# T1uTiu/ProDiff

Measured on AMD Instinct MI355X. Metric: mel-frames/sec + audio RTF, 2-iter ProDiff + 4-iter FastDiff @1/2/4/8 GPU, higher is better.
Workload: dtype bf16; 1 GPU; C3: ProDiff 2-iter (WaveNet 20x256, M=80, vpsde max_beta 40) + FastDiff 4-iter (base.yaml, hop 256), 8 x 861-frame utterances per GPU; global_batch=8, per_gpu_batch=8, seq_len=861, batches_per_gpu=1, jobs_in_flight=2, schedule=job i on HIP stream i % 2, parallelism=dp1 (utterance shards, RCCL gather to rank 0)

## Files before the change

### include/prodiff_hip.h

```cpp
#ifndef PRODIFF_HIP_H
#define PRODIFF_HIP_H

#include <stddef.h>

#ifdef __cplusplus
extern "C" {
#endif

#define PD_OK 0
#define PD_ERR_ARG 1
#define PD_ERR_HIP 2
#define PD_ERR_WORKSPACE 3
#define PD_ERR_UNSUPPORTED 4

#define PD_DTYPE_F32 0
#define PD_DTYPE_BF16 1

const char* pd_last_error(void);
int pd_version(void);
const char* pd_build_config(void);
size_t pd_live_device_bytes(void);

int pd_profile_enable(int on);
int pd_profile_summary(char* buf, int buflen);
// ... 55 lines not shown
  int inner_channels;
  int cond_channels;
  int num_blocks;
  int upsample_ratios[4];
  int lvc_layers_each_block;
  int lvc_kernel_size;
  int kpnet_hidden_channels;
  int kpnet_conv_size;
  int step_embed_in;
  int step_embed_mid;
  int step_embed_out;
} fd_dims;

#define FD_NUM_PARAMS(nb) (2 + 4 + 30 * (nb) + 8 * (nb) + 2)

int fd_create(const fd_dims* dims, const float* const* params, int dtype, void* stream,
              fd_model** out);
void fd_destroy(fd_model* m);
int fd_hop(const fd_model* m);
size_t fd_workspace_size(const fd_model* m, int B, int Tc, int S);

#define FD_OPT_LVC_TS 0
#define FD_OPT_LVC_TS_SUB 1
#define FD_OPT_LVC_FUSE 2
#define FD_OPT_LVC_PF 3
#define FD_OPT_LVC_SUB 4
#define FD_OPT_KP_SIDE 5
#define FD_OPT_KP_CHUNK 7
#define FD_OPT_LVC_TPW 10
#define FD_OPT_LVC_PRIO 11
#define FD_OPT_LVC_PS 14
#define FD_OPT_LVC_CARRY 15
#define FD_OPT_LVC_PS_GRID 16
int fd_set_option(fd_model* m, int option, int value);

int fd_lvc_ps_partition(int rows, int batch, int grid, int* runs, int cap, int* nruns);

int fd_fold_weight_norm(float* w, const float* g, const float* v, int cout, int per_row,
                        void* stream);

int fd_forward(const fd_model* m, const float* audio, const float* cond, const float* steps,
               float* eps, int B, int Tc, void* workspace, size_t ws_bytes, void* stream);

int fd_sample(const fd_model* m, const float* mel, const float* beta, const float* alpha,
              const float* sigma, const float* steps, int N, const float* x_T,
              const float* noise, unsigned long long seed, const int* utt_ids, const int* lens, float* wav,
              int B, int Tc, void* workspace, size_t ws_bytes, void* stream);

int fd_sample_coefs(const fd_model* m, const float* mel, const float* ce, const float* den,
                    const float* sg, const float* steps, int N, const float* x_T,
                    const float* noise, unsigned long long seed, const int* utt_ids, const int* lens,
                    int draw0, float* wav, int B, int Tc, void* workspace, size_t ws_bytes, void* stream);

int fd_draw_x_T(const fd_model* m, float* x_T, int B, int Tc, unsigned long long seed, const int* utt_ids,
                void* stream);

typedef struct nsf_model nsf_model;

typedef struct {
  int num_mels;
  int upsample_initial_channel;
  int num_upsamples;
  int upsample_rates[6];
  int upsample_kernel_sizes[6];
  int resblock;
  int num_kernels;
  int resblock_kernel_sizes[4];
  int num_dilations;
  int resblock_dilation_sizes[4][4];
// ... 278 lines not shown
```

### prodiff_amd/_lib.py

```python
from __future__ import annotations

import ctypes as C
import os

_HERE = os.path.dirname(os.path.abspath(__file__))
LIB_PATH = os.environ.get("PRODIFF_HIP_LIB", os.path.join(_HERE, "libprodiff_hip.so"))

PD_DTYPE_F32 = 0
PD_DTYPE_BF16 = 1
PD_REFLOW = {"euler": 0, "rk2": 1, "rk4": 2, "rk5": 3}
FD_OPTIONS = {"lvc_ts": 0, "lvc_ts_sub": 1, "lvc_fuse": 2, "lvc_pf": 3, "lvc_sub": 4, "kp_side": 5, "kp_chunk": 7,
               "lvc_tpw": 10, "lvc_prio": 11, "lvc_ps": 14, "lvc_carry": 15, "lvc_ps_grid": 16}
NSF_OPTIONS = {"small_max": 0, "wconv": 1, "pair": 2, "pair16": 3, "ups_nc": 4, "rb16": 5, "rb32": 6, "rb64": 7, "c256": 8, "nc_mfma": 9}
WN_OPTIONS = {"layer": 0, "ksplit": 1, "l2pf": 2, "stack": 3, "stack_ro": 4, "stack_fuse": 6, "f32_layer": 7}


class HipError(RuntimeError):
    pass


class pd_wavenet_dims(C.Structure):
    _fields_ = [("in_dims", C.c_int), ("hidden_size", C.c_int), ("residual_layers", C.c_int),
                ("residual_channels", C.c_int), ("dilation_cycle_length", C.c_int)]


class fd_dims(C.Structure):
    _fields_ = [("audio_channels", C.c_int), ("inner_channels", C.c_int),
                ("cond_channels", C.c_int), ("num_blocks", C.c_int),
                ("upsample_ratios", C.c_int * 4), ("lvc_layers_each_block", C.c_int),
                ("lvc_kernel_size", C.c_int), ("kpnet_hidden_channels", C.c_int),
                ("kpnet_conv_size", C.c_int), ("step_embed_in", C.c_int),
                ("step_embed_mid", C.c_int), ("step_embed_out", C.c_int)]


class nsf_dims(C.Structure):
    _fields_ = [("num_mels", C.c_int), ("upsample_initial_channel", C.c_int), ("num_upsamples", C.c_int),
                ("upsample_rates", C.c_int * 6), ("upsample_kernel_sizes", C.c_int * 6), ("resblock", C.c_int),
                ("num_kernels", C.c_int), ("resblock_kernel_sizes", C.c_int * 4), ("num_dilations", C.c_int),
                ("resblock_dilation_sizes", (C.c_int * 4) * 4), ("sampling_rate", C.c_int),
                ("harmonic_num", C.c_int)]


class pd_cond_dims(C.Structure):
    _fields_ = [("vocab_size", C.c_int), ("hidden_size", C.c_int), ("enc_layers", C.c_int),
                ("enc_ffn_kernel_size", C.c_int), ("num_heads", C.c_int), ("num_spk", C.c_int),
# ... 56 lines not shown

class pd_curves_dims(C.Structure):
    _fields_ = [("samplerate", C.c_int), ("win_size", C.c_int), ("hop_size", C.c_int), ("half_width", C.c_float)]


_VP = C.c_void_p
_SIGS = {
    "pd_last_error": (C.c_char_p, []),
    "pd_version": (C.c_int, []),
    "pd_build_config": (C.c_char_p, []),
    "pd_live_device_bytes": (C.c_size_t, []),
    "pd_profile_enable": (C.c_int, [C.c_int]),
    "pd_profile_summary": (C.c_int, [C.c_char_p, C.c_int]),
    "pd_profile_filter": (C.c_int, [C.c_char_p]),
    "pd_wavenet_create": (C.c_int, [C.POINTER(pd_wavenet_dims), C.POINTER(_VP), C.c_int, _VP, C.POINTER(_VP)]),
    "pd_wavenet_destroy": (None, [_VP]),
    "pd_wavenet_set_option": (C.c_int, [_VP, C.c_int, C.c_int]),
    "pd_wavenet_workspace_size": (C.c_size_t, [_VP, C.c_int, C.c_int, C.c_int]),
    "pd_wavenet_forward": (C.c_int, [_VP, _VP, _VP, _VP, _VP, C.c_int, C.c_int, _VP, C.c_size_t, _VP]),
    "pd_prodiff_sample": (C.c_int, [_VP, _VP, C.POINTER(C.c_float), C.POINTER(C.c_float),
                                    C.POINTER(C.c_float), C.c_int, _VP, _VP, C.c_ulonglong, _VP, _VP, _VP,
                                    C.c_int, C.c_int, _VP, C.c_size_t, _VP]),
    "pd_reflow_workspace_size": (C.c_size_t, [_VP, C.c_int, C.c_int, C.c_int, C.c_int]),
    "pd_reflow_sample": (C.c_int, [_VP, _VP, C.c_int, C.c_int, C.c_float, _VP, C.c_ulonglong, _VP, _VP, _VP,
                                   C.c_int, C.c_int, _VP, C.c_size_t, _VP]),
    "pd_reflow_denorm": (C.c_int, [_VP, _VP, _VP, C.c_int, C.c_int, C.c_int, C.c_int, C.c_float, C.c_float,
                                   _VP, _VP]),
    "fd_create": (C.c_int, [C.POINTER(fd_dims), C.POINTER(_VP), C.c_int, _VP, C.POINTER(_VP)]),
    "fd_destroy": (None, [_VP]),
    "fd_hop": (C.c_int, [_VP]),
    "fd_workspace_size": (C.c_size_t, [_VP, C.c_int, C.c_int, C.c_int]),
    "fd_set_option": (C.c_int, [_VP, C.c_int, C.c_int]),
    "fd_lvc_ps_partition": (C.c_int, [C.c_int, C.c_int, C.c_int, C.POINTER(C.c_int), C.c_int, C.POINTER(C.c_int)]),
    "fd_fold_weight_norm": (C.c_int, [_VP, _VP, _VP, C.c_int, C.c_int, _VP]),
    "fd_forward": (C.c_int, [_VP, _VP, _VP, _VP, _VP, C.c_int, C.c_int, _VP, C.c_size_t, _VP]),
    "fd_sample": (C.c_int, [_VP, _VP, C.POINTER(C.c_float), C.POINTER(C.c_float), C.POINTER(C.c_float),
                            C.POINTER(C.c_float), C.c_int, _VP, _VP, C.c_ulonglong, _VP, _VP, _VP, C.c_int,
                            C.c_int, _VP, C.c_size_t, _VP]),
    "fd_sample_coefs": (C.c_int, [_VP, _VP, C.POINTER(C.c_float), C.POINTER(C.c_float), C.POINTER(C.c_float),
                                  C.POINTER(C.c_float), C.c_int, _VP, _VP, C.c_ulonglong, _VP, _VP, C.c_int, _VP,
                                  C.c_int, C.c_int, _VP, C.c_size_t, _VP]),
    "fd_draw_x_T": (C.c_int, [_VP, _VP, C.c_int, C.c_int, C.c_ulonglong, _VP, _VP]),
    "pd_cond_num_params": (C.c_int, [C.POINTER(pd_cond_dims)]),
    "pd_cond_create": (C.c_int, [C.POINTER(pd_cond_dims), C.POINTER(_VP), C.c_int, _VP, C.POINTER(_VP)]),
    "pd_cond_destroy": (None, [_VP]),
    "pd_cond_workspace_size": (C.c_size_t, [_VP, C.c_int, C.c_int, C.c_int]),
    "pd_cond_forward": (C.c_int, [_VP, C.POINTER(pd_cond_inputs), _VP, _VP, C.c_int, C.c_int, C.c_int, _VP,
                                  C.c_size_t, _VP]),
    "pd_pitch_cond_num_params": (C.c_int, [C.POINTER(pd_pitch_cond_dims)]),
    "pd_pitch_cond_create": (C.c_int, [C.POINTER(pd_pitch_cond_dims), C.POINTER(_VP), C.c_int, _VP, C.POINTER(_VP)]),
    "pd_pitch_cond_destroy": (None, [_VP]),
    "pd_pitch_cond_workspace_size": (C.c_size_t, [_VP, C.c_int, C.c_int, C.c_int, C.c_int]),
    "pd_pitch_cond_forward": (C.c_int, [_VP, C.POINTER(pd_pitch_cond_inputs), _VP, C.c_int, C.c_int, C.c_int,
                                        C.c_int, _VP, C.c_size_t, _VP]),
    "pd_dur_num_params": (C.c_int, [C.POINTER(pd_dur_dims)]),
    "pd_dur_create": (C.c_int, [C.POINTER(pd_dur_dims), C.POINTER(_VP), C.c_int, _VP, C.POINTER(_VP)]),
    "pd_dur_destroy": (None, [_VP]),
    "pd_dur_workspace_size": (C.c_size_t, [_VP, C.c_int, C.c_int]),
    "pd_dur_forward": (C.c_int, [_VP, C.POINTER(pd_dur_inputs), _VP, _VP, C.c_int, C.c_int, _VP, C.c_size_t, _VP]),
    "nsf_num_params": (C.c_int, [C.POINTER(nsf_dims)]),
    "nsf_create": (C.c_int, [C.POINTER(nsf_dims), C.POINTER(_VP), C.c_int, _VP, C.POINTER(_VP)]),
    "nsf_destroy": (None, [_VP]),
    "nsf_hop": (C.c_int, [_VP]),
    "nsf_workspace_size": (C.c_size_t, [_VP, C.c_int, C.c_int]),
    "nsf_set_option": (C.c_int, [_VP, C.c_int, C.c_int]),
    "nsf_forward": (C.c_int, [_VP, _VP, C.c_float, _VP, _VP, _VP, C.c_ulonglong, _VP, _VP, _VP, C.c_int, C.c_int,
# ... 349 lines not shown
```

### prodiff_amd/csrc/fastdiff.hip

```cpp
#include <cmath>
#include <vector>

#include "../../include/prodiff_hip.h"
#include "gemm.h"
#include "kernels.h"

using namespace pd;

namespace {
constexpr int CI = 32;
constexpr int CC = 80;
constexpr int HK = 64;
constexpr int NLY = 4;
constexpr int KPERLAYER = 2 * CI * CI * 3;
constexpr int EMB_IN = 128, EMB_MID = 512, EMB_OUT = 512;
constexpr int FD_STEP_CHUNK = 16;

__host__ __device__ inline int lvc_pos(int ci) { return (((ci >> 2) & 1) << 4) | ((ci >> 3) << 2) | (ci & 3); }
__host__ __device__ inline int lvc_chan(int p) { return (p & 3) | (((p & 15) >> 2) << 3) | ((p >> 4) << 2); }
__host__ __device__ inline int kf_packed(int o, int q) {
  const int k = (q & ~31) | lvc_pos(q & 31);
  return (((o >> 5) * 6 + (k >> 4)) * 64 + ((k & 15) >> 3) * 32 + (o & 31)) * 8 + (k & 7);
}
__host__ __device__ inline void kf_unpack(int p, int& o, int& q) {
  const int j = p & 7, l = (p >> 3) & 63, kkn = p >> 9;
  o = (kkn / 6) * 32 + (l & 31);
  const int k = (kkn % 6) * 16 + (l >> 5) * 8 + j;
  q = (k & ~31) | lvc_chan(k & 31);
}
}

struct fd_model {
  int nblocks;
  int ratios[4];
  int hops[4];
  int dtype;
  int lvc_ts = 384;
  int lvc_ts_sub = 256;
  bool lvc_fuse = true;
  bool lvc_pf = true;
  bool lvc_sub = true;
  bool kp_side = false;
  int kp_chunk = 0;
  int lvc_tpw = 2;
  int lvc_prio = 0;
  int lvc_ps = 1;
  int lvc_carry = 1;
  int lvc_ps_grid = 0;

  mutable hipStream_t side = nullptr;
  mutable hipEvent_t ev_hidden = nullptr, ev_kp[4] = {}, ev_lvc[4] = {};
  WeightPool weights;
  DevBuf kps;
  float *fc1_w, *fc1_b, *fc2_w, *fc2_b;
  float *first_w, *first_b;
  float *final_w, *final_b;
  struct Block {
    float *up_w, *up_b;
    float *upf_w;
    float *fct_w, *fct_b;
    float *kin_w, *kin_b;
    float *kres_w[6], *kres_b[6];
    float *kk_w, *kk_b;
    __bf16* kks_w = nullptr;
    float* kks_b = nullptr;
    float *kb_w, *kb_b;
    float *cv_w[NLY], *cv_b[NLY];
  } blk[4];
  struct Down {
    float *c0_w, *c0_b, *c1_w, *c1_b;
    float *c2_w, *c2_b;
  } dn[4];

  ~fd_model() {
    if (side) {
      (void)hipStreamSynchronize(side);
      (void)hipStreamDestroy(side);
    }
    if (ev_hidden) (void)hipEventDestroy(ev_hidden);
    for (int n = 0; n < 4; ++n) {
      if (ev_kp[n]) (void)hipEventDestroy(ev_kp[n]);
// ... 206 lines not shown
      const int s = mt * 32 + (reg & 3) + 8 * (reg >> 2) + 4 * h;
      const long long idx = (base + t0 + s) * CI + r32;
      x[idx] = x[idx] + a[idx] + gate_fast(ag[reg] + bg, afl[reg] + bl);
    }
  }
}

struct LvcBlockArgs {
  float* xout;
  const float* xin;
  const float* a;
  const __bf16* Kf[NLY];
  const float* Bf;
  const __bf16* Wc[NLY];
  const float* bc[NLY];
  const __bf16* Wup;
  const float* bup;
  int r, p;
  const float* audio;
  const float* fw;
  const float* fb;
  const float* wfin;
  const float* bfin;
  float* audio_out;
  const float* noise;
  float ce, den, sig;
  unsigned long long seed;
  unsigned stream;
  const int* uid;
  int Tc, hop;
  const int* lens;
  int b_off;
  int prio;
#ifdef LB_TRACE
  unsigned long long* trace;
#endif
};
#ifdef LB_TRACE
#define LB_STAMP(i)                                                                       \
  do {                                                                                    \
    if (lane == 0 && blockIdx.x % 61 == 0)                                                \
      P.trace[((blockIdx.y * gridDim.x + blockIdx.x) / 61 * NW + wave) * 24 + (i)] =      \
          __builtin_readcyclecounter();                                                   \
  } while (0)
#else
#define LB_STAMP(i) \
  do {              \
  } while (0)
#endif
constexpr int LB_LD = 40;
constexpr int LB_XLD = 36;
template <int TS, int TPW = 2> struct LbGeo {
  static constexpr int NG = TS / 32 + 4;
  static constexpr int NW = NG / TPW;
  static constexpr int NT = NW * 64;
  static constexpr int UOFF = 28;
  static constexpr int UROWS = NG * 32 + 2 * UOFF;
  static constexpr int YROWS = (NG + 1) * 32;
  static constexpr int UY_BYTES = (UROWS + YROWS) * LB_LD * 2;
  static constexpr int XS_BYTES = NG * 32 * LB_XLD * 4;
  static constexpr int NTJ_MAX = (NG * 32 / 4 + 2 + 31) / 32;
  static constexpr int XP_BYTES = (NTJ_MAX * 32 + 1) * LB_LD * 2;
  static constexpr int SMEM = UY_BYTES > XS_BYTES + XP_BYTES ? UY_BYTES : XS_BYTES + XP_BYTES;
};

#ifdef LVC_SCALAR_F32
// ... 1 lines not shown
__device__ __forceinline__ f32x2 operator+(f32x2 a, f32x2 b) { return f32x2{a.x + b.x, a.y + b.y}; }
__device__ __forceinline__ f32x2 operator-(f32x2 a, f32x2 b) { return f32x2{a.x - b.x, a.y - b.y}; }
__device__ __forceinline__ f32x2 operator*(f32x2 a, f32x2 b) { return f32x2{a.x * b.x, a.y * b.y}; }
__device__ __forceinline__ f32x2 operator+(f32x2 a, float b) { return f32x2{a.x + b, a.y + b}; }
__device__ __forceinline__ f32x2 operator*(f32x2 a, float b) { return f32x2{a.x * b, a.y * b}; }
__device__ __forceinline__ f32x2& operator+=(f32x2& a, f32x2 b) { a = a + b; return a; }
__device__ __forceinline__ f32x2 efma(f32x2 a, f32x2 b, f32x2 c) { return f32x2{fmaf(a.x, b.x, c.x), fmaf(a.y, b.y, c.y)}; }
__device__ __forceinline__ f32x2 emax(f32x2 a, f32x2 b) {
  return f32x2{__builtin_elementwise_maximum(a.x, b.x), __builtin_elementwise_maximum(a.y, b.y)};
}
#else
typedef float f32x2 __attribute__((ext_vector_type(2)));
__device__ __forceinline__ f32x2 efma(f32x2 a, f32x2 b, f32x2 c) { return __builtin_elementwise_fma(a, b, c); }
__device__ __forceinline__ f32x2 emax(f32x2 a, f32x2 b) { return __builtin_elementwise_maximum(a, b); }
#endif
constexpr float LOG2E = 1.4426950408889634f;
__device__ __forceinline__ f32x2 lrelu2(f32x2 v) {
  const f32x2 s = v * 0.2f;
  return emax(v, s);
}
__device__ __forceinline__ f32x2 gate2ef(f32x2 fs) {
  constexpr float C = 15.f * 2.f * LOG2E;
  return f32x2{__builtin_amdgcn_exp2f(__builtin_amdgcn_fmed3f(fs.x, -C, C)),
               __builtin_amdgcn_exp2f(__builtin_amdgcn_fmed3f(fs.y, -C, C))};
}
__device__ __forceinline__ f32x2 gate2r(f32x2 gs, f32x2 fs) {
  const f32x2 ef = gate2ef(fs);
  const f32x2 eg1 = f32x2{__builtin_amdgcn_exp2f(gs.x), __builtin_amdgcn_exp2f(gs.y)} + 1.f;
  const f32x2 den = efma(ef, eg1, eg1);
  return f32x2{__builtin_amdgcn_rcpf(den.x), __builtin_amdgcn_rcpf(den.y)};
}
__device__ __forceinline__ int floordiv(int a, int b) { return (a >= 0 ? a : a - b + 1) / b; }

template <int TS, bool UPS, bool AUD, bool FIN, bool PF = false, bool SUB = false, int TPW = 2>
__global__ __launch_bounds__((LbGeo<TS, TPW>::NT), (TPW == 1 ? LbGeo<TS, TPW>::NT / 256 : (PF || SUB) ? 2 : 3))
void lvc_block_bf16_kernel(const LvcBlockArgs P) {
  static_assert(!(PF && SUB), "prefetch assumes one frame per tile");
  static_assert(TPW == 1 || TPW == 2, "one or two tiles per wave");
  using G = LbGeo<TS, TPW>;
  constexpr int NW = G::NW, NG = G::NG, UOFF = G::UOFF, GR = NG * 32;
  constexpr int EX = FIN ? 3 : 0;
  __shared__ __attribute__((aligned(16))) char smem[G::SMEM];
  __shared__ float AS[AUD ? GR + 6 : 1];
  __shared__ __attribute__((aligned(16))) float FW[AUD ? 7 * 32 : 4];
  __shared__ __attribute__((aligned(16))) float FWF[FIN ? 7 * 32 : 4];
  __shared__ __attribute__((aligned(16))) float FBL[AUD ? 32 : 4];
  __shared__ __attribute__((aligned(16))) float BUL[UPS ? 32 : 4];
  constexpr bool WL = PF, WW = PF || SUB;
  constexpr int BFR = WL ? GR / 64 + 2 : 1;
  __shared__ __attribute__((aligned(16))) bf16x8 WCL[WW ? NLY * 6 * 64 : 1];
  __shared__ __attribute__((aligned(16))) float BCL[WW ? NLY * CI : 4];
  __shared__ __attribute__((aligned(16))) float BFL[WL ? BFR * 2 * CI * NLY : 4];
  __bf16* U = reinterpret_cast<__bf16*>(smem);
  __bf16* Y = U + G::UROWS * LB_LD;
  float* XS = reinterpret_cast<float*>(smem);
  __bf16* XP = reinterpret_cast<__bf16*>(smem + G::XS_BYTES);
  const int tid = threadIdx.x, lane = tid & 63, wave = tid >> 6, n = lane & 31, h = lane >> 5;
  int bx, b;
  {
    const int total = gridDim.x * gridDim.y, id = blockIdx.y * gridDim.x + blockIdx.x;
    const int xcd = id & 7, slot = id >> 3, per = total >> 3, rem = total & 7;
    const int logical = xcd < rem ? xcd * (per + 1) + slot : rem * (per + 1) + (xcd - rem) * per + slot;
    b = logical / gridDim.x;
    bx = logical - b * gridDim.x;
  }
  const int jsw = !PF && (bx & 1);
#define TILE(j) (TPW == 1 ? wave : PF ? 2 * wave + (j) : wave + ((j) ^ jsw) * NW)
  const int Tc = P.Tc, hop = P.hop;
  const int Lh = Tc * hop;
  const int Le = P.lens ? min(P.lens[b], Tc) * hop : Lh;
  const int t0 = bx * TS, tg = t0 - 64;
  const long long base = (long long)b * Lh;
  constexpr int RLO = 64 - 44 - EX, RHI = 64 + TS + 44 + EX;
  LB_STAMP(0);
  const int fbase = (tg > 0 ? tg : 0) / hop;
  constexpr int IT = AUD ? (GR + 6 + G::NT - 1) / G::NT : 1;
  float av[IT], fwv = 0.f, fbv = 0.f, bupv = 0.f, wfv = 0.f;
  if constexpr (AUD) {
#pragma unroll
    for (int it = 0; it < IT; ++it) {
      const int t = tg - 3 + tid + it * G::NT;
      av[it] = P.audio[base + min(max(t, 0), Lh - 1)];
    }
    if (tid < 224) fwv = P.fw[(tid & 31) * 7 + (tid >> 5)];
    if (tid < 32) fbv = P.fb[tid];
  }
  if constexpr (UPS) {
    if (tid < 32) bupv = P.bup[tid];
  }
  if constexpr (FIN) {
    if (tid < 224) wfv = P.wfin[tid];
  }
  constexpr int IW = WW ? (6 * 64 + G::NT - 1) / G::NT : 1;
  constexpr int N4 = BFR * 2 * CI * NLY / 4, IB = WL ? (N4 + G::NT - 1) / G::NT : 1;
  bf16x4 wv[IW][NLY][2];
  float bcv = 0.f;
  float4 bfv[IB];
  if constexpr (WW) {
#pragma unroll
    for (int it = 0; it < IW; ++it) {
      const int i = min(tid + it * G::NT, 6 * 64 - 1), kk = i >> 6, ln = i & 63;
#pragma unroll
      for (int l = 0; l < NLY; ++l) {
        const __bf16* w = P.Wc[l] + (ln & 31) * 96 + (kk >> 1) * 32 + 16 * (ln >> 5) + 4 * (kk & 1);
        wv[it][l][0] = *reinterpret_cast<const bf16x4*>(w);
        wv[it][l][1] = *reinterpret_cast<const bf16x4*>(w + 8);
      }
    }
    if (tid < NLY * CI) {
#pragma unroll
      for (int l = 0; l < NLY; ++l)
        if (tid / CI == l) bcv = P.bc[l][tid % CI];
    }
  }
  if constexpr (WL) {
#pragma unroll
    for (int it = 0; it < IB; ++it) {
      const int i = min(tid + it * G::NT, N4 - 1), fr = min(fbase + i / (2 * CI * NLY / 4), Tc - 1);
      const int c = (i % (2 * CI * NLY / 4)) * 4;
      bfv[it] = *reinterpret_cast<const float4*>(P.Bf + ((long long)b * Tc + fr) * (2 * CI * NLY) + c);
    }
  }
  const int r = UPS ? P.r : 1, pp = UPS ? P.p : 0, Tin = Lh / r, Tin_e = Le / r;
  const int ntj = (GR / r + 2 + 31) / 32;
  const int jb = floordiv(tg + pp, r) - 2;
  constexpr int IX = UPS ? ((G::NTJ_MAX * 32 + 1) * 8 + G::NT - 1) / G::NT : 1;
  float4 xv4[IX];
  const bool by_phase = NW % r == 0 && ntj <= 4 * (NW / r);
  bf16x8 wfj[4][4];
  auto wup_load = [&](int job0) {
    if (by_phase) {
      const __bf16* wa = P.Wup + ((long long)(wave % r) * 32 + n) * 64 + 8 * h;
#pragma unroll
      for (int kk = 0; kk < 4; ++kk) wfj[0][kk] = *reinterpret_cast<const bf16x8*>(wa + kk * 16);
      return;
    }
#pragma unroll
    for (int q = 0; q < 4; ++q) {
      const int job = job0 + q * NW, k = job / ntj;
      if (job < r * ntj) {
        const __bf16* wa = P.Wup + ((long long)k * 32 + n) * 64 + 8 * h;
#pragma unroll
        for (int kk = 0; kk < 4; ++kk) wfj[q][kk] = *reinterpret_cast<const bf16x8*>(wa + kk * 16);
      }
    }
  };
  if constexpr (UPS) {
    const float* xp = P.xin + (long long)b * Tin * CI;
#pragma unroll
    for (int it = 0; it < IX; ++it) {
      const int i = tid + it * G::NT, q = (i & 7) * 4, j = min(max(jb + (i >> 3), 0), Tin - 1);
      xv4[it] = *reinterpret_cast<const float4*>(xp + (long long)j * CI + q);
    }
// ... 27 lines not shown
      const int t = tg - 3 + i;
      if (i < GR + 6) AS[i] = (t >= 0 && t < Le) ? av[it] : 0.f;
    }
    if (tid < 224) FW[tid] = fwv;
    if (tid < 32) FBL[tid] = fbv;
  }
  if constexpr (UPS) {
    if (tid < 32) BUL[tid] = bupv;
  }
  if constexpr (FIN) {
    if (tid < 224) FWF[tid] = wfv;
  }
  if constexpr (WW) {
#pragma unroll
    for (int it = 0; it < IW; ++it) {
      const int i = tid + it * G::NT;
#pragma unroll
      for (int l = 0; l < NLY; ++l) {
        const bf16x4 w0 = wv[it][l][0], w1 = wv[it][l][1];
        if (i < 6 * 64) WCL[l * 384 + i] = bf16x8{w0[0], w0[1], w0[2], w0[3], w1[0], w1[1], w1[2], w1[3]};
      }
    }
    if (tid < NLY * CI) BCL[tid] = bcv;
  }
  if constexpr (WL) {
#pragma unroll
    for (int it = 0; it < IB; ++it) {
      const int i = tid + it * G::NT, c = (i % (2 * CI * NLY / 4)) * 4;
      const float sc = fbase + i / (2 * CI * NLY / 4) >= Tc ? 0.f : (c & 63) < 32 ? -LOG2E : 2.f * LOG2E;
      if (i < N4)
        *reinterpret_cast<float4*>(&BFL[4 * i]) = make_float4(bfv[it].x * sc, bfv[it].y * sc, bfv[it].z * sc, bfv[it].w * sc);
    }
  }
  LB_STAMP(16);
  f32x2 xr[TPW][8], ar[TPW][8];
  if constexpr (UPS) {
#pragma unroll
    for (int it = 0; it < IX; ++it) {
      const int i = tid + it * G::NT, rr = i >> 3, q = (i & 7) * 4, j = jb + rr;
      if (i < (ntj * 32 + 1) * 8) {
        const float m = (j >= 0 && j < Tin_e) ? 1.f : 0.f;
        const f32x2 u0 = lrelu2(f32x2{xv4[it].x, xv4[it].y} * m), u1 = lrelu2(f32x2{xv4[it].z, xv4[it].w} * m);
        *reinterpret_cast<bf16x4*>(&XP[rr * LB_LD + q]) = bf16x4{(__bf16)u0.x, (__bf16)u0.y, (__bf16)u1.x, (__bf16)u1.y};
      }
    }
    __syncthreads();
    LB_STAMP(17);
    for (int job0 = wave; job0 < r * ntj; job0 += 4 * NW) {
    if (job0 != wave && !by_phase) wup_load(job0);
#pragma unroll
    for (int q = 0; q < 4; ++q) {
      int k, jt;
      if (by_phase) {
        k = wave % r; jt = wave / r + q * (NW / r);
        if (jt >= ntj) break;
      } else {
        const int job = job0 + q * NW;
        if (job >= r * ntj) break;
        k = job / ntj; jt = job - k * ntj;
      }
      f32x16 acc;
#pragma unroll
      for (int i = 0; i < 16; ++i) acc[i] = 0.f;
#pragma unroll
      for (int kk = 0; kk < 4; ++kk) {
        const bf16x8 xb = *reinterpret_cast<const bf16x8*>(
// ... 27 lines not shown
      if (ok) {
        if constexpr (UPS) xv = *reinterpret_cast<const float4*>(&XS[row * LB_XLD + 8 * i + 4 * h]);
        else xv = *reinterpret_cast<const float4*>(P.xin + (base + t) * CI + 8 * i + 4 * h);
        if constexpr (AUD) {
          float a4[4];
#pragma unroll
          for (int e = 0; e < 4; ++e) a4[e] = FBL[8 * i + 4 * h + e];
#pragma unroll
          for (int tap = 0; tap < 7; ++tap) {
            const float s = AS[row + tap];
            const float4 w = *reinterpret_cast<const float4*>(&FW[tap * 32 + 8 * i + 4 * h]);
            a4[0] = fmaf(w.x, s, a4[0]); a4[1] = fmaf(w.y, s, a4[1]);
            a4[2] = fmaf(w.z, s, a4[2]); a4[3] = fmaf(w.w, s, a4[3]);
          }
          av = make_float4(a4[0], a4[1], a4[2], a4[3]);
        } else {
          av = *reinterpret_cast<const float4*>(P.a + (base + t) * CI + 8 * i + 4 * h);
        }
      }
      xr[j][2 * i] = f32x2{xv.x + av.x, xv.y + av.y}; xr[j][2 * i + 1] = f32x2{xv.z + av.z, xv.w + av.w};
      ar[j][2 * i] = f32x2{av.x, av.y}; ar[j][2 * i + 1] = f32x2{av.z, av.w};
    }
  }
  LB_STAMP(19);
  if constexpr (UPS) __syncthreads();
  if constexpr (!PF) {
    const bf16x8 z = {};
    for (int i = tid; i < G::UY_BYTES / 16; i += G::NT) reinterpret_cast<bf16x8*>(smem)[i] = z;
  }
  LB_STAMP(20);
  __syncthreads();
  LB_STAMP(1);
  if (P.prio && wave >= NW / 2) __builtin_amdgcn_s_setprio(1);
#pragma unroll
  for (int l = 0; l < NLY; ++l) {
    const int d = l == 0 ? 1 : l == 1 ? 3 : l == 2 ? 9 : 27;
    const int e = (l == 0 ? 42 : l == 1 ? 38 : l == 2 ? 28 : 0) + EX;
    const int kf = (64 - e) / 32, kl = (64 + TS + e - 1) / 32;
    const int kpl = kl + 1 < NG - 1 ? kl + 1 : NG - 1;
#pragma unroll
    for (int j = 0; j < TPW; ++j) {
      const int k = TILE(j);
      if (k >= kf - 1 && k <= kl + 2) {
        bf16x8 u0, u1;
#pragma unroll
        for (int p = 0; p < 4; ++p) {
          const f32x2 v0 = lrelu2(xr[j][p]), v1 = lrelu2(xr[j][4 + p]);
          u0[2 * p] = (__bf16)v0.x; u0[2 * p + 1] = (__bf16)v0.y;
          u1[2 * p] = (__bf16)v1.x; u1[2 * p + 1] = (__bf16)v1.y;
        }
        if constexpr (PF) {
          const int ts = tg + k * 32;
          if (ts < 0 || ts >= Le) { u0 = bf16x8{}; u1 = bf16x8{}; }
        }
        __bf16* dst = &U[(k * 32 + n + UOFF) * LB_LD + 16 * h];
        *reinterpret_cast<bf16x8*>(dst) = u0;
        *reinterpret_cast<bf16x8*>(dst + 8) = u1;
      }
    }
    __syncthreads();
    LB_STAMP(2 + 3 * l);
    {
      bf16x8 wf[6];
#pragma unroll
      for (int kk = 0; kk < 6; ++kk) {
        if constexpr (WW) {
          wf[kk] = WCL[(l * 6 + kk) * 64 + lane];
        } else {
          const __bf16* w = P.Wc[l] + n * 96 + (kk >> 1) * 32 + 16 * h + 4 * (kk & 1);
          const bf16x4 w0 = *reinterpret_cast<const bf16x4*>(w), w1 = *reinterpret_cast<const bf16x4*>(w + 8);
          wf[kk] = bf16x8{w0[0], w0[1], w0[2], w0[3], w1[0], w1[1], w1[2], w1[3]};
// ... 109 lines not shown
#pragma unroll
      for (int j = 0; j < TPW; ++j) gate_update(j, g[j], f[j], nullptr, true);
    } else {
#pragma unroll
    for (int j = 0; j < TPW; ++j) {
      const int k = TILE(j), ts = tg + k * 32;
      if (k >= kf && k <= kl && ts >= 0 && ts < Le) {
        f32x16 g, f;
#pragma unroll
        for (int r = 0; r < 16; ++r) { g[r] = 0.f; f[r] = 0.f; }
        const float* bq;
        if constexpr (SUB) {
          const int f0 = ts / hop, fn = (ts + n) / hop;
          const int nf = min(32 / hop, Tc - f0);
          const __bf16* kq0 = P.Kf[l] + ((long long)b * Tc + f0) * KPERLAYER;
          bf16x8 ka[12], kb[12];
          auto kld = [&](bf16x8 (&d)[12], int i) {
            const __bf16* kq = kq0 + (long long)min(i, nf - 1) * KPERLAYER;
#pragma unroll
            for (int kk = 0; kk < 12; ++kk) d[kk] = *reinterpret_cast<const bf16x8*>(kq + (kk * 64 + lane) * 8);
            __builtin_amdgcn_sched_barrier(0);
          };
          auto kmm = [&](const bf16x8 (&kf)[12], int i) {
            const bool mine = fn == f0 + i;
#pragma unroll
            for (int kk = 0; kk < 6; ++kk) {
              const bf16x8 yv = *reinterpret_cast<const bf16x8*>(&Y[(k * 32 + n + (kk >> 1)) * LB_LD + 16 * (kk & 1) + 8 * h]);
              const bf16x8 z = {};
              const bf16x8 ym = mine ? yv : z;
              g = __builtin_amdgcn_mfma_f32_32x32x16_bf16(kf[kk], ym, g, 0, 0, 0);
              f = __builtin_amdgcn_mfma_f32_32x32x16_bf16(kf[6 + kk], ym, f, 0, 0, 0);
            }
          };
          kld(ka, 0);
          for (int i = 0; i < nf; i += 2) {
            kld(kb, i + 1);
            kmm(ka, i);
            if (i + 1 < nf) {
              kld(ka, i + 2);
              kmm(kb, i + 1);
            }
          }
          bq = P.Bf + ((long long)b * Tc + (fn < Tc ? fn : Tc - 1)) * (2 * CI * NLY) + l * 2 * CI;
        } else {
          const int frame = ts / hop;
          const __bf16* kq = P.Kf[l] + ((long long)b * Tc + frame) * KPERLAYER;
          bq = P.Bf + ((long long)b * Tc + frame) * (2 * CI * NLY) + l * 2 * CI;
#pragma unroll
          for (int kk = 0; kk < 6; ++kk) {
            const int tap = kk >> 1;
            const bf16x8 yb = *reinterpret_cast<const bf16x8*>(&Y[(k * 32 + n + tap) * LB_LD + 16 * (kk & 1) + 8 * h]);
            const bf16x8 kg = *reinterpret_cast<const bf16x8*>(kq + (kk * 64 + lane) * 8);
            const bf16x8 kt = *reinterpret_cast<const bf16x8*>(kq + ((6 + kk) * 64 + lane) * 8);
            g = __builtin_amdgcn_mfma_f32_32x32x16_bf16(kg, yb, g, 0, 0, 0);
            f = __builtin_amdgcn_mfma_f32_32x32x16_bf16(kt, yb, f, 0, 0, 0);
          }
        }
        float4 bb[8];
#pragma unroll
        for (int i = 0; i < 4; ++i) {
          bb[i] = *reinterpret_cast<const float4*>(bq + 8 * i + 4 * h);
          bb[4 + i] = *reinterpret_cast<const float4*>(bq + 32 + 8 * i + 4 * h);
        }
        __builtin_amdgcn_sched_barrier(0);
        gate_update(j, g, f, bb, !SUB || ts + n < Le);
      }
    }
    }
    if (l < NLY - 1) LB_STAMP(4 + 3 * l);
  }
  LB_STAMP(14);
  if constexpr (FIN) {
    float* E = XS;
    __syncthreads();
#pragma unroll
    for (int j = 0; j < TPW; ++j) {
// ... 14 lines not shown
#pragma unroll
        for (int tap = 0; tap < 7; ++tap) st[tap] += __shfl_xor(st[tap], 32);
        if constexpr (PF) {
          const int ts = tg + k * 32;
          if (ts < 0 || ts >= Le) {
#pragma unroll
            for (int tap = 0; tap < 7; ++tap) st[tap] = 0.f;
          }
        }
        if (h == 0) {
          *reinterpret_cast<float4*>(&E[row * 8]) = make_float4(st[0], st[1], st[2], st[3]);
          *reinterpret_cast<float4*>(&E[row * 8 + 4]) = make_float4(st[4], st[5], st[6], 0.f);
        }
      }
    }
    __syncthreads();
    constexpr int IS = (TS + G::NT - 1) / G::NT;
#pragma unroll
    for (int it = 0; it < IS; ++it) {
      const int s = tid + it * G::NT, t = t0 + s;
      if (s < TS && t < Lh) {
        float e = bfin;
#pragma unroll
        for (int tap = 0; tap < 7; ++tap) e += E[(64 + s + tap - 3) * 8 + tap];
        float v = (AS[67 + s] - P.ce * e) / P.den;
        if (P.sig != 0.f) v += P.sig * zr[it];
        P.audio_out[base + t] = v;
      }
    }
  } else {
#pragma unroll
    for (int j = 0; j < TPW; ++j) {
      const int k = TILE(j), t = tg + k * 32 + n;
      if (k >= 2 && k < 2 + TS / 32 && t < Lh) {
#pragma unroll
        for (int i = 0; i < 4; ++i)
          *reinterpret_cast<float4*>(P.xout + (base + t) * CI + 8 * i + 4 * h) =
              make_float4(xr[j][2 * i].x, xr[j][2 * i].y, xr[j][2 * i + 1].x, xr[j][2 * i + 1].y);
      }
    }
  }
  LB_STAMP(15);
#undef TILE
}

#pragma clang diagnostic push
#pragma clang diagnostic ignored "-Winline-asm"
__device__ __forceinline__ void lds_dma16(const void* g, void* lds) {
  const unsigned l = __builtin_amdgcn_readfirstlane((unsigned)(size_t)lds);
  asm volatile("s_mov_b32 m0, %0\n\tglobal_load_lds_dwordx4 %1, off" ::"s"(l), "v"(g) : "memory", "m0");
}
__device__ __forceinline__ void lds_dma4(const void* g, void* lds) {
  const unsigned l = __builtin_amdgcn_readfirstlane((unsigned)(size_t)lds);
  asm volatile("s_mov_b32 m0, %0\n\tglobal_load_lds_dword %1, off" ::"s"(l), "v"(g) : "memory", "m0");
}
#pragma clang diagnostic pop
__host__ __device__ inline void lvc_ps_run(int rn, int nruns, int batch, int rows, int& b, int& t0, int& t1) {
  b = ((rn + 1) * batch - 1) / nruns;
  const int first = b * nruns / batch, n = (b + 1) * nruns / batch - first, i = rn - first;
  const long long units = (rows + 63) / 64;
  t0 = (int)(i * units / n) * 64;
  t1 = i + 1 == n ? rows : (int)((i + 1) * units / n) * 64;
}
static inline int lvc_ps_grid(int rows, int batch, int ncu, int cap, int* nruns_carry) {
  const int ntiles = (int)cdiv(rows, 384) * batch;
  int grid = ntiles <= ncu ? ntiles : ncu >= 8 ? ncu / 8 * 8 : ncu;
  if (cap > 0 && cap < grid) grid = cap;
// ... 1256 lines not shown
  float* xn;
  const float* ad;
  const float* Bfp;
};

int launch_lvc_ps(const fd_model* m, const LvcBlockArgs& la, bool fin, long long Tout, int B, hipStream_t st) {
  int dev = 0, ncu = 0;
  PD_HIP(hipGetDevice(&dev));
  PD_HIP(hipDeviceGetAttribute(&ncu, hipDeviceAttributeMultiprocessorCount, dev));
  const int ntx = (int)cdiv(Tout, 384), ntiles = ntx * B;
  int nruns = 0;
  const int grid = lvc_ps_grid((int)Tout, B, ncu, m->lvc_ps_grid, &nruns);
  const int nb = m->lvc_carry && nruns ? B : 0;
  if (!nb) nruns = ntiles;
  dispatch([&](auto FINAL) {
    hipLaunchKernelGGL(lvc_ps_kernel<FINAL()>, dim3(grid), dim3(512), 0, st, la, ntx, nruns, nb);
  }, bool_of(fin));
  PD_LAUNCH_CHECK();
  return PD_OK;
}

int launch_lvc_block(const fd_model* m, const LvcBlockArgs& la, bool ups, bool aud, bool fin, long long Tout, int B,
                     hipStream_t st) {
  const int hop = la.hop, ts = hop < 32 ? m->lvc_ts_sub : m->lvc_ts;
  const bool pf = m->lvc_pf && hop % 64 == 0;
  const bool ps_fin = fin && la.r == 4 && hop % 256 == 0;
  const bool ps_ups = ups && !fin && !aud && la.a && la.r == 8 && hop % 64 == 0;
  if (pf && ts == 384 && m->lvc_tpw == 2 && m->lvc_ps && (ps_fin || ps_ups)) return launch_lvc_ps(m, la, ps_fin, Tout, B, st);
  auto go = [&](auto TS, auto UPS, auto AUD, auto FIN, auto PF, auto SUB, auto TPW) {
    hipLaunchKernelGGL((lvc_block_bf16_kernel<TS(), UPS(), AUD(), FIN(), PF(), SUB(), TPW()>), dim3(cdiv(Tout, TS()), B),
                       dim3(LbGeo<TS(), TPW()>::NT), 0, st, la);
  };
  const bool sub = hop < 32;
  if (ts == 384 && m->lvc_tpw == 1 && !sub && ups && aud == fin) {
    dispatch([&](auto FIN, auto PF) { go(Const<384>{}, Const<true>{}, FIN, FIN, PF, Const<false>{}, Const<1>{}); },
             bool_of(fin), bool_of(pf));
    PD_LAUNCH_CHECK();
    return PD_OK;
  }
  if (sub && (aud || fin)) { set_error("lvc_block: audio/final fusion needs hop >= 32"); return PD_ERR_ARG; }
  if (!ups && (aud || fin)) { set_error("lvc_block: audio/final fusion needs the fused upsample"); return PD_ERR_ARG; }
  if (fin && !aud) { set_error("lvc_block: final fusion needs the audio fusion"); return PD_ERR_ARG; }
  const bool pfk = pf && !sub && ups && aud == fin;
  dispatch([&](auto TS) {
    dispatch_rows<DispatchRow<false, false, false, false, true>, DispatchRow<true, false, false, false, true>,
                  DispatchRow<false, false, false, false, false>, DispatchRow<true, false, false, false, false>,
                  DispatchRow<true, false, false, true, false>, DispatchRow<true, true, false, false, false>,
                  DispatchRow<true, true, true, false, false>, DispatchRow<true, true, true, true, false>>(
        [&](auto... cs) { go(TS, cs..., Const<2>{}); }, ups, aud, fin, pfk, sub);
  }, one_of<128, 256, 384>(ts == 256 || ts == 384 ? ts : 128));
  PD_LAUNCH_CHECK();
  return PD_OK;
}

int fd_downsample(const FdCall& c, const float* downs[4], const float** bottom) {
  const fd_model* m = c.m;
  const int nb = m->nblocks;
  const long long L = (long long)c.Tc * m->hops[nb - 1];
  float* a0 = c.ws + c.W.a0;
  if (!c.aud) {
    ProfScope ps("fd_first_conv", c.st);
    hipLaunchKernelGGL(first_conv_kernel, dim3(cdiv(L, 32), c.B), dim3(256), 0, c.st, c.xa, m->first_w,
                       m->first_b, a0, (int)L, c.lens, m->hops[nb - 1]);
    PD_LAUNCH_CHECK();
  }
  const float* cur = a0;
// ... 366 lines not shown
      return PD_OK;
    case FD_OPT_LVC_TS_SUB:
      PD_CHECK_ARG(value == 128 || value == 256 || value == 384, "FD_OPT_LVC_TS_SUB in {128,256,384}");
      m->lvc_ts_sub = value;
      return PD_OK;
    case FD_OPT_LVC_FUSE: m->lvc_fuse = value != 0; return PD_OK;
    case FD_OPT_LVC_PF: m->lvc_pf = value != 0; return PD_OK;
    case FD_OPT_LVC_SUB: m->lvc_sub = value != 0; return PD_OK;
    case FD_OPT_KP_SIDE: m->kp_side = value != 0; return PD_OK;
    case FD_OPT_KP_CHUNK:
      PD_CHECK_ARG(value >= 0, "FD_OPT_KP_CHUNK >= 0");
      m->kp_chunk = value;
      return PD_OK;
    case FD_OPT_LVC_PRIO:
      PD_CHECK_ARG(value == 0 || value == 1, "FD_OPT_LVC_PRIO in {0,1}");
      m->lvc_prio = value;
      return PD_OK;
    case FD_OPT_LVC_PS:
      PD_CHECK_ARG(value == 0 || value == 1, "FD_OPT_LVC_PS in {0,1}");
      m->lvc_ps = value;
      return PD_OK;
    case FD_OPT_LVC_TPW:
      PD_CHECK_ARG(value == 1 || value == 2, "FD_OPT_LVC_TPW in {1,2}");
      m->lvc_tpw = value;
      return PD_OK;
    case FD_OPT_LVC_CARRY:
      PD_CHECK_ARG(value == 0 || value == 1, "FD_OPT_LVC_CARRY in {0,1}");
      m->lvc_carry = value;
      return PD_OK;
    case FD_OPT_LVC_PS_GRID:
      PD_CHECK_ARG(value >= 0, "FD_OPT_LVC_PS_GRID >= 0");
      m->lvc_ps_grid = value;
      return PD_OK;
    default: break;
  }
  set_error("fd_set_option: unknown option " + std::to_string(option));
  return PD_ERR_ARG;
}

int fd_lvc_ps_partition(int rows, int batch, int grid, int* runs, int cap, int* nruns) {
  PD_CHECK_ARG(nruns && rows > 0 && rows % 64 == 0 && batch > 0 && grid > 0,
               "rows (a multiple of 64), batch and grid must be positive");
  PD_CHECK_ARG((long long)batch * (rows / 64) < (1ll << 24), "launch too large");
  lvc_ps_grid(rows, batch, 1 << 30, grid, nruns);
  for (int i = 0; runs && i < *nruns && i < cap; ++i)
    lvc_ps_run(i, *nruns, batch, rows, runs[3 * i], runs[3 * i + 1], runs[3 * i + 2]);
  return PD_OK;
}

int fd_forward(const fd_model* m, const float* audio, const float* cond, const float* steps, float* eps,
               int B, int Tc, void* workspace, size_t ws_bytes, void* stream) {
  PD_CHECK_ARG(m && audio && cond && steps && eps && workspace, "null pointer");
  PD_CHECK_ARG(B > 0 && Tc > 0, "B and T' must be positive");
  FdWs W = fd_layout(m, B, Tc, 1);
  if (ws_bytes < W.total) { set_error("workspace too small"); return PD_ERR_WORKSPACE; }
  hipStream_t st = (hipStream_t)stream;
  float* ws = (float*)workspace;
  const long long L = (long long)Tc * m->hops[m->nblocks - 1];
  PD_HIP(hipMemcpyAsync(ws + W.steps, steps, sizeof(float) * B, hipMemcpyDeviceToDevice, st));
  PD_TRY(fd_step_mlp(m, ws, W, B, st));
  PD_TRY(transpose_ct_to_tc(cond, ws + W.condT, B, CC, Tc, st));
  float* x = nullptr;
  if (m->weights.bf16()) PD_TRY(fd_kp_hidden_all(m, ws, W, ws + W.condT, ws + W.nz, 1, B, Tc, st));
  PD_TRY(fd_net(m, ws, W, audio, ws + W.condT, ws + W.nz, 0, B, Tc, &x, st));
  hipLaunchKernelGGL(final_conv_kernel, dim3(cdiv(L, 256), B), dim3(256), 0, st, x, m->final_w, m->final_b,
                     eps, (float*)nullptr, 0.f, 0.f, 0.f, (const float*)nullptr, 0ull, 0u, (const int*)nullptr, L,
                     (const int*)nullptr, 1);
  PD_LAUNCH_CHECK();
  return PD_OK;
}

int fd_sample_coefs(const fd_model* m, const float* mel, const float* ce_, const float* den_, const float* sg_,
                    const float* steps_, int N, const float* x_T, const float* noise, unsigned long long seed,
                    const int* utt_ids, const int* lens, int draw0, float* wav, int B, int Tc, void* workspace,
                    size_t ws_bytes, void* stream) {
  PD_CHECK_ARG(m && mel && ce_ && den_ && sg_ && steps_ && wav && workspace, "null pointer");
  PD_CHECK_ARG(B > 0 && Tc > 0 && N >= 1 && draw0 >= 0, "bad B/T'/N/draw0");
  const int CH = N < FD_STEP_CHUNK ? N : FD_STEP_CHUNK;
  FdWs W = fd_layout(m, B, Tc, CH);
// ... 123 lines not shown
```

Baseline: 1.657 million mel-frames/s.

## Add run-partitioned hop-8 LVC block kernel with staged bias and kernel prefetch

Adds a new path for the hop-8 upsampled LVC block that splits each utterance's rows into variable-length runs, sized to the CU count and rounded to multiples of 32. Each workgroup covers one run instead of a fixed tile. Inside the kernel, per-frame bias rows are staged into shared memory, and the next layer's kernel-predictor weights are prefetched into registers while the current layer's MFMA work runs. The aim is less tail imbalance and less global-load latency in the sub-32-hop block, at the cost of more registers and LDS and a dynamic tile size.

```diff
diff --git a/include/prodiff_hip.h b/include/prodiff_hip.h
--- a/include/prodiff_hip.h
+++ b/include/prodiff_hip.h
@@ -111,9 +111,11 @@
 #define FD_OPT_LVC_PS 14
 #define FD_OPT_LVC_CARRY 15
 #define FD_OPT_LVC_PS_GRID 16
+#define FD_OPT_LVC_SUB_PS 17
 int fd_set_option(fd_model* m, int option, int value);
 
 int fd_lvc_ps_partition(int rows, int batch, int grid, int* runs, int cap, int* nruns);
+int fd_lvc_sub_partition(int rows, int batch, int ts, int grid, int* runs, int cap, int* nruns);
 
 int fd_fold_weight_norm(float* w, const float* g, const float* v, int cout, int per_row,
                         void* stream);
diff --git a/prodiff_amd/_lib.py b/prodiff_amd/_lib.py
--- a/prodiff_amd/_lib.py
+++ b/prodiff_amd/_lib.py
@@ -10,7 +10,8 @@
 PD_DTYPE_BF16 = 1
 PD_REFLOW = {"euler": 0, "rk2": 1, "rk4": 2, "rk5": 3}
 FD_OPTIONS = {"lvc_ts": 0, "lvc_ts_sub": 1, "lvc_fuse": 2, "lvc_pf": 3, "lvc_sub": 4, "kp_side": 5, "kp_chunk": 7,
-               "lvc_tpw": 10, "lvc_prio": 11, "lvc_ps": 14, "lvc_carry": 15, "lvc_ps_grid": 16}
+               "lvc_tpw": 10, "lvc_prio": 11, "lvc_ps": 14, "lvc_carry": 15, "lvc_ps_grid": 16,
+               "lvc_sub_ps": 17}
 NSF_OPTIONS = {"small_max": 0, "wconv": 1, "pair": 2, "pair16": 3, "ups_nc": 4, "rb16": 5, "rb32": 6, "rb64": 7, "c256": 8, "nc_mfma": 9}
 WN_OPTIONS = {"layer": 0, "ksplit": 1, "l2pf": 2, "stack": 3, "stack_ro": 4, "stack_fuse": 6, "f32_layer": 7}
 
@@ -133,6 +134,8 @@
     "fd_workspace_size": (C.c_size_t, [_VP, C.c_int, C.c_int, C.c_int]),
     "fd_set_option": (C.c_int, [_VP, C.c_int, C.c_int]),
     "fd_lvc_ps_partition": (C.c_int, [C.c_int, C.c_int, C.c_int, C.POINTER(C.c_int), C.c_int, C.POINTER(C.c_int)]),
+    "fd_lvc_sub_partition": (C.c_int, [C.c_int, C.c_int, C.c_int, C.c_int, C.POINTER(C.c_int), C.c_int,
+                                       C.POINTER(C.c_int)]),
     "fd_fold_weight_norm": (C.c_int, [_VP, _VP, _VP, C.c_int, C.c_int, _VP]),
     "fd_forward": (C.c_int, [_VP, _VP, _VP, _VP, _VP, C.c_int, C.c_int, _VP, C.c_size_t, _VP]),
     "fd_sample": (C.c_int, [_VP, _VP, C.POINTER(C.c_float), C.POINTER(C.c_float), C.POINTER(C.c_float),
diff --git a/prodiff_amd/csrc/fastdiff.hip b/prodiff_amd/csrc/fastdiff.hip
--- a/prodiff_amd/csrc/fastdiff.hip
+++ b/prodiff_amd/csrc/fastdiff.hip
@@ -47,6 +47,7 @@
   int lvc_ps = 1;
   int lvc_carry = 1;
   int lvc_ps_grid = 0;
+  int lvc_sub_ps = 1;
 
   mutable hipStream_t side = nullptr;
   mutable hipEvent_t ev_hidden = nullptr, ev_kp[4] = {}, ev_lvc[4] = {};
@@ -319,6 +320,7 @@
   const int* lens;
   int b_off;
   int prio;
+  int sub_runs, sub_nb;
 #ifdef LB_TRACE
   unsigned long long* trace;
 #endif
@@ -386,10 +388,28 @@
 }
 __device__ __forceinline__ int floordiv(int a, int b) { return (a >= 0 ? a : a - b + 1) / b; }
 
-template <int TS, bool UPS, bool AUD, bool FIN, bool PF = false, bool SUB = false, int TPW = 2>
+__host__ __device__ inline void lvc_sub_run(int rn, int nruns, int batch, int rows, int& b, int& t0, int& t1) {
+  b = (int)((((long long)rn + 1) * batch - 1) / nruns);
+  const int first = (int)((long long)b * nruns / batch), n = (int)(((long long)b + 1) * nruns / batch) - first;
+  const int i = rn - first;
+  const long long units = (rows + 31) / 32;
+  t0 = (int)(i * units / n) * 32;
+  t1 = i + 1 == n ? rows : (int)((i + 1) * units / n) * 32;
+}
+static inline int lvc_sub_nruns(int rows, int batch, int ts, int ncu, int cap, bool fine) {
+  const long long units = (rows + 31) / 32, most = units * batch, least = (units + ts / 32 - 1) / (ts / 32) * batch;
+  const long long all = ncu >= 8 ? ncu / 8 * 8 : ncu;
+  long long want = cap > 0 ? cap : fine && 2 * least <= all ? all : least;
+  if (want > most) want = most;
+  if (want < least) want = least;
+  return (int)want;
+}
+
+template <int TS, bool UPS, bool AUD, bool FIN, bool PF = false, bool SUB = false, int TPW = 2, bool RUN = false>
 __global__ __launch_bounds__((LbGeo<TS, TPW>::NT), (TPW == 1 ? LbGeo<TS, TPW>::NT / 256 : (PF || SUB) ? 2 : 3))
 void lvc_block_bf16_kernel(const LvcBlockArgs P) {
   static_assert(!(PF && SUB), "prefetch assumes one frame per tile");
+  static_assert(!RUN || (SUB && UPS && !AUD && !FIN && TPW == 2), "runs: the hop-8 block only");
   static_assert(TPW == 1 || TPW == 2, "one or two tiles per wave");
   using G = LbGeo<TS, TPW>;
   constexpr int NW = G::NW, NG = G::NG, UOFF = G::UOFF, GR = NG * 32;
@@ -405,27 +425,41 @@
   __shared__ __attribute__((aligned(16))) bf16x8 WCL[WW ? NLY * 6 * 64 : 1];
   __shared__ __attribute__((aligned(16))) float BCL[WW ? NLY * CI : 4];
   __shared__ __attribute__((aligned(16))) float BFL[WL ? BFR * 2 * CI * NLY : 4];
+  constexpr int NFR = GR / 8;
+  __shared__ __attribute__((aligned(16))) float BFS[RUN ? NFR * 2 * CI * NLY : 4];
   __bf16* U = reinterpret_cast<__bf16*>(smem);
   __bf16* Y = U + G::UROWS * LB_LD;
   float* XS = reinterpret_cast<float*>(smem);
   __bf16* XP = reinterpret_cast<__bf16*>(smem + G::XS_BYTES);
   const int tid = threadIdx.x, lane = tid & 63, wave = tid >> 6, n = lane & 31, h = lane >> 5;
   int bx, b;
+  int t0 = 0, TSr = TS;
   {
     const int total = gridDim.x * gridDim.y, id = blockIdx.y * gridDim.x + blockIdx.x;
     const int xcd = id & 7, slot = id >> 3, per = total >> 3, rem = total & 7;
     const int logical = xcd < rem ? xcd * (per + 1) + slot : rem * (per + 1) + (xcd - rem) * per + slot;
-    b = logical / gridDim.x;
-    bx = logical - b * gridDim.x;
+    if constexpr (RUN) {
+      int rb, r0, r1;
+      lvc_sub_run(logical, P.sub_runs, P.sub_nb, P.Tc * P.hop, rb, r0, r1);
+      b = __builtin_amdgcn_readfirstlane(rb);
+      bx = logical;
+      t0 = __builtin_amdgcn_readfirstlane(r0);
+      TSr = __builtin_amdgcn_readfirstlane((r1 - r0 + 31) / 32 * 32);
+    } else {
+      b = logical / gridDim.x;
+      bx = logical - b * gridDim.x;
+      t0 = bx * TS;
+    }
   }
   const int jsw = !PF && (bx & 1);
 #define TILE(j) (TPW == 1 ? wave : PF ? 2 * wave + (j) : wave + ((j) ^ jsw) * NW)
   const int Tc = P.Tc, hop = P.hop;
   const int Lh = Tc * hop;
   const int Le = P.lens ? min(P.lens[b], Tc) * hop : Lh;
-  const int t0 = bx * TS, tg = t0 - 64;
+  const int tg = t0 - 64;
   const long long base = (long long)b * Lh;
-  constexpr int RLO = 64 - 44 - EX, RHI = 64 + TS + 44 + EX;
+  constexpr int RLO = 64 - 44 - EX;
+  const int RHI = 64 + TSr + 44 + EX;
   LB_STAMP(0);
   const int fbase = (tg > 0 ? tg : 0) / hop;
   constexpr int IT = AUD ? (GR + 6 + G::NT - 1) / G::NT : 1;
@@ -473,6 +507,15 @@
       const int i = min(tid + it * G::NT, N4 - 1), fr = min(fbase + i / (2 * CI * NLY / 4), Tc - 1);
       const int c = (i % (2 * CI * NLY / 4)) * 4;
       bfv[it] = *reinterpret_cast<const float4*>(P.Bf + ((long long)b * Tc + fr) * (2 * CI * NLY) + c);
+    }
+  }
+  constexpr int IS4 = RUN ? (NFR * 2 * CI * NLY / 4 + G::NT - 1) / G::NT : 1;
+  float4 bsv[IS4];
+  if constexpr (RUN) {
+#pragma unroll
+    for (int it = 0; it < IS4; ++it) {
+      const int i = min(tid + it * G::NT, NFR * 2 * CI * NLY / 4 - 1), fr = min(fbase + i / (2 * CI * NLY / 4), Tc - 1);
+      bsv[it] = *reinterpret_cast<const float4*>(P.Bf + ((long long)b * Tc + fr) * (2 * CI * NLY) + (i % (2 * CI * NLY / 4)) * 4);
     }
   }
   const int r = UPS ? P.r : 1, pp = UPS ? P.p : 0, Tin = Lh / r, Tin_e = Le / r;
@@ -566,6 +609,13 @@
         *reinterpret_cast<float4*>(&BFL[4 * i]) = make_float4(bfv[it].x * sc, bfv[it].y * sc, bfv[it].z * sc, bfv[it].w * sc);
     }
   }
+  if constexpr (RUN) {
+#pragma unroll
+    for (int it = 0; it < IS4; ++it) {
+      const int i = tid + it * G::NT;
+      if (i < NFR * 2 * CI * NLY / 4) *reinterpret_cast<float4*>(&BFS[4 * i]) = bsv[it];
+    }
+  }
   LB_STAMP(16);
   f32x2 xr[TPW][8], ar[TPW][8];
   if constexpr (UPS) {
@@ -659,11 +709,35 @@
   __syncthreads();
   LB_STAMP(1);
   if (P.prio && wave >= NW / 2) __builtin_amdgcn_s_setprio(1);
+  auto lvc_on = [&](int ll, int jj) {
+    const int e = (ll == 0 ? 42 : ll == 1 ? 38 : ll == 2 ? 28 : 0) + EX;
+    const int k = TILE(jj), ts = tg + k * 32;
+    return k >= (64 - e) / 32 && k <= (64 + TSr + e - 1) / 32 && ts >= 0 && ts < Le;
+  };
+  auto kfirst = [&](int ll, int jj) {
+    return P.Kf[ll] + ((long long)b * Tc + max(tg + TILE(jj) * 32, 0) / hop) * KPERLAYER;
+  };
+  auto knext = [&](int l0, int j0) {
+    const __bf16* p = P.Kf[0] + (long long)b * Tc * KPERLAYER;
+#pragma unroll
+    for (int ll = NLY - 1; ll >= 0; --ll) {
+#pragma unroll
+      for (int jj = TPW - 1; jj >= 0; --jj)
+        if ((ll > l0 || (ll == l0 && jj > j0)) && lvc_on(ll, jj)) p = kfirst(ll, jj);
+    }
+    return p;
+  };
+  bf16x8 kc[RUN ? 12 : 1];
+  if constexpr (RUN) {
+    const __bf16* kq = knext(-1, 0);
+#pragma unroll
+    for (int kk = 0; kk < 12; ++kk) kc[kk] = *reinterpret_cast<const bf16x8*>(kq + (kk * 64 + lane) * 8);
+  }
 #pragma unroll
   for (int l = 0; l < NLY; ++l) {
     const int d = l == 0 ? 1 : l == 1 ? 3 : l == 2 ? 9 : 27;
     const int e = (l == 0 ? 42 : l == 1 ? 38 : l == 2 ? 28 : 0) + EX;
-    const int kf = (64 - e) / 32, kl = (64 + TS + e - 1) / 32;
+    const int kf = (64 - e) / 32, kl = (64 + TSr + e - 1) / 32;
     const int kpl = kl + 1 < NG - 1 ? kl + 1 : NG - 1;
 #pragma unroll
     for (int j = 0; j < TPW; ++j) {
@@ -839,6 +913,22 @@
               f = __builtin_amdgcn_mfma_f32_32x32x16_bf16(kf[6 + kk], ym, f, 0, 0, 0);
             }
           };
+          if constexpr (RUN) {
+            kld(kb, 1);
+            kmm(kc, 0);
+            kld(kc, 2);
+            if (1 < nf) kmm(kb, 1);
+            kld(kb, 3);
+            if (2 < nf) kmm(kc, 2);
+            bq = &BFS[((fn < Tc ? fn : Tc - 1) - fbase) * (2 * CI * NLY) + l * 2 * CI];
+            {
+              const __bf16* kq = knext(l, j);
+#pragma unroll
+              for (int kk = 0; kk < 12; ++kk) kc[kk] = *reinterpret_cast<const bf16x8*>(kq + (kk * 64 + lane) * 8);
+              __builtin_amdgcn_sched_barrier(0);
+            }
+            if (3 < nf) kmm(kb, 3);
+          } else {
           kld(ka, 0);
           for (int i = 0; i < nf; i += 2) {
             kld(kb, i + 1);
@@ -849,6 +939,7 @@
             }
           }
           bq = P.Bf + ((long long)b * Tc + (fn < Tc ? fn : Tc - 1)) * (2 * CI * NLY) + l * 2 * CI;
+          }
         } else {
           const int frame = ts / hop;
           const __bf16* kq = P.Kf[l] + ((long long)b * Tc + frame) * KPERLAYER;
@@ -929,7 +1020,7 @@
 #pragma unroll
     for (int j = 0; j < TPW; ++j) {
       const int k = TILE(j), t = tg + k * 32 + n;
-      if (k >= 2 && k < 2 + TS / 32 && t < Lh) {
+      if (k >= 2 && k < 2 + TSr / 32 && t < Lh) {
 #pragma unroll
         for (int i = 0; i < 4; ++i)
           *reinterpret_cast<float4*>(P.xout + (base + t) * CI + 8 * i + 4 * h) =
@@ -2252,6 +2343,21 @@
                        dim3(LbGeo<TS(), TPW()>::NT), 0, st, la);
   };
   const bool sub = hop < 32;
+  if (sub && hop == 8 && ups && !aud && !fin && m->lvc_sub_ps && ts != 384) {
+    int dev = 0, ncu = 0;
+    PD_HIP(hipGetDevice(&dev));
+    PD_HIP(hipDeviceGetAttribute(&ncu, hipDeviceAttributeMultiprocessorCount, dev));
+    const int tsr = ts == 256 ? 256 : 128;
+    LvcBlockArgs lr = la;
+    lr.sub_runs = lvc_sub_nruns((int)Tout, B, tsr, ncu, m->lvc_ps_grid, m->lvc_sub_ps == 2);
+    lr.sub_nb = B;
+    dispatch([&](auto TS) {
+      hipLaunchKernelGGL((lvc_block_bf16_kernel<TS(), true, false, false, false, true, 2, true>), dim3(lr.sub_runs),
+                         dim3(LbGeo<TS(), 2>::NT), 0, st, lr);
+    }, one_of<128, 256>(tsr));
+    PD_LAUNCH_CHECK();
+    return PD_OK;
+  }
   if (ts == 384 && m->lvc_tpw == 1 && !sub && ups && aud == fin) {
     dispatch([&](auto FIN, auto PF) { go(Const<384>{}, Const<true>{}, FIN, FIN, PF, Const<false>{}, Const<1>{}); },
              bool_of(fin), bool_of(pf));
@@ -2684,6 +2790,10 @@
       PD_CHECK_ARG(value >= 0, "FD_OPT_LVC_PS_GRID >= 0");
       m->lvc_ps_grid = value;
       return PD_OK;
+    case FD_OPT_LVC_SUB_PS:
+      PD_CHECK_ARG(value >= 0 && value <= 2, "FD_OPT_LVC_SUB_PS in {0,1,2}");
+      m->lvc_sub_ps = value;
+      return PD_OK;
     default: break;
   }
   set_error("fd_set_option: unknown option " + std::to_string(option));
@@ -2697,6 +2807,16 @@
   lvc_ps_grid(rows, batch, 1 << 30, grid, nruns);
   for (int i = 0; runs && i < *nruns && i < cap; ++i)
     lvc_ps_run(i, *nruns, batch, rows, runs[3 * i], runs[3 * i + 1], runs[3 * i + 2]);
+  return PD_OK;
+}
+
+int fd_lvc_sub_partition(int rows, int batch, int ts, int grid, int* runs, int cap, int* nruns) {
+  PD_CHECK_ARG(nruns && rows > 0 && rows % 8 == 0 && batch > 0 && grid > 0 && (ts == 128 || ts == 256),
+               "rows (a multiple of 8), batch and grid must be positive, ts 128 or 256");
+  PD_CHECK_ARG((long long)batch * ((rows + 31) / 32) < (1ll << 24), "launch too large");
+  *nruns = lvc_sub_nruns(rows, batch, ts, 0, grid, false);
+  for (int i = 0; runs && i < *nruns && i < cap; ++i)
+    lvc_sub_run(i, *nruns, batch, rows, runs[3 * i], runs[3 * i + 1], runs[3 * i + 2]);
   return PD_OK;
 }
 
```

New measurement: 1.661 million mel-frames/s (median of 4 runs). No clear change (+0.3%).
